# yanjunzan/GMAT

Measured on AMD Instinct MI355X. Metric: SNP-pairs tested/sec (whole node) + GRM GFLOP/s, mouse-sized cohort, higher is better.
Workload: dtype fp6xfp4/fp64

## Files before the change

gmat_amd/_native.py:

```python
import ctypes
import os

import numpy as np

_HERE = os.path.dirname(os.path.abspath(__file__))
LIB_PATH = os.environ.get("GMAT_HIP_LIB", os.path.join(_HERE, "libgmat_hip.so"))

GMAT_AA, GMAT_AD, GMAT_DD = 0, 1, 2
GMAT_GRM_ADD, GMAT_GRM_DOM = 0, 1
GMAT_SCREEN_NONE = -9

_P = ctypes.c_void_p
_I64 = ctypes.c_int64
_D = ctypes.c_double
_INT = ctypes.c_int

_PROTOS = {
    "gmat_last_error": (ctypes.c_char_p, []),
    "gmat_version": (_INT, []),
    "gmat_device_count": (_INT, [_P]),
    "gmat_set_device": (_INT, [_INT]),
    "gmat_device_synchronize": (_INT, []),
    "gmat_empty_cache": (_INT, []),
    "gmat_reml_stats": (_INT, [_P]),
    "gmat_reml_trace": (_INT, [_INT, _P, _P, _P, _P]),
    "gmat_epi_setup_stats": (_INT, [_P, _P]),
    "gmat_geno_create": (_INT, [_P, _P, _I64, _I64, _I64]),
    "gmat_geno_counts": (_INT, [_P, _P, _P, _P]),
    "gmat_geno_destroy": (_INT, [_P]),
    "gmat_grm": (_INT, [_P, _INT, _D, _P, _P]),
    "gmat_grm_stats": (_INT, [_P]),
    "gmat_spd_inverse": (_INT, [_I64, _P, _P, _P]),
    "gmat_reml": (_INT, [_I64, _I64, _I64, _INT, _P, _P, _P, _P, _P, _INT, _D, _D, _P, _P, _P]),
    "gmat_projection": (_INT, [_I64, _I64, _I64, _INT, _P, _P, _P, _P, _P, _P, _P]),
    "gmat_epi_create": (_INT, [_P, _P, _P, _P, _INT]),
    "gmat_epi_create_with": (_INT, [_P, _P, _P, _P, _INT, _P, _I64]),
    "gmat_epi_export": (_INT, [_P, _P, _I64, _P]),
    "gmat_epi_scan": (_INT, [_P, _INT, _P, _I64, _D, _D, _INT, _P]),
    "gmat_epi_hits": (_INT, [_P, _I64, _P, _P, _P, _P, _P, _P]),
    "gmat_epi_pairs": (_INT, [_P, _INT, _P, _I64, _P, _P, _P, _P]),
    "gmat_epi_stats": (_INT, [_P, _P]),
    "gmat_epi_audit": (_INT, [_P, _INT, _P, _I64, _P]),
    "gmat_epi_kernel_stats": (_INT, [_P, _P]),
    "gmat_epi_kernel_stats_ext": (_INT, [_P, _P, _INT, _P]),
    "gmat_epi_info": (_INT, [_P, _P]),
    "gmat_epi_layout": (_INT, [_P, _P]),
    "gmat_epi_destroy": (_INT, [_P]),
    "gmat_eff_scan": (_INT, [_P, _INT, _P, _P, _I64, _P, _P, _P, ctypes.c_char_p, _P]),
    "gmat_eff_stats": (_INT, [_P]),
    "gmat_geno_decode": (_INT, [_P, _P]),
    "gmat_blup": (_INT, [_I64, _I64, _I64, _INT, _P, _P, _P, _P, _P, _P]),
    "gmat_write_grm_text": (_INT, [ctypes.c_char_p, _P, _I64, _INT, ctypes.c_char_p, _INT]),
    "gmat_float_repr": (_INT, [_D, ctypes.c_char_p, _INT]),
    "gmat_append_hit_rows": (_INT, [ctypes.c_char_p, _I64, _P, _P, _INT, _P, _P, _P, _P]),
    "gmat_snp_test": (_INT, [_P, _INT, _P, _P, _P, _P]),
    "gmat_lmm_snp_test": (_INT, [_P, _INT, _P, _P, _I64, _P, _P, _P]),
    "gmat_lmm_epi_rows": (_INT, [_P, _P, _I64, _I64, _P, _P, _P, _P]),
    "gmat_lmm_stats": (_INT, [_P]),
    "gmat_probe_mx_accum":(_INT, [_INT, _P, _P, _P]),
    "gmat_probe_eig_bottom": (_INT, [_I64, _P, _INT, _D, _INT, _P, _P, _P, _P]),
    "gmat_probe_dgemm": (_INT, [_I64, _I64, _I64, _D, _D, _INT, _P, _INT, _INT, _I64, _P, _INT, _INT, _I64, _P, _I64]),
    "gmat_probe_cholesky": (_INT, [_I64, _P, _I64, _INT, _P, _P, _P, _P, _P, _P]),
    "gmat_probe_dot_rows": (_INT, [_I64, _I64, _P, _I64, _P, _I64, _P]),
    "gmat_comm_unique_id": (_INT, [_P]),
    "gmat_comm_init": (_INT, [_P, _INT, _INT, _P]),
    "gmat_comm_destroy": (_INT, [_P]),
    "gmat_comm_allgather": (_INT, [_P, _P, _P, _I64]),
    "gmat_comm_broadcast": (_INT, [_P, _P, _I64, _INT]),
    "gmat_comm_allreduce_f64": (_INT, [_P, _P, _I64, _INT]),
    "gmat_comm_gatherv": (_INT, [_P, _P, _I64, _INT, _P, _P, _I64, _P]),
    "gmat_comm_barrier": (_INT, [_P]),
    "read_plink_bed": (_INT, [ctypes.c_char_p, _I64, _I64, _P]),
    "remma_epiAA_eff_cpu": (_INT, [ctypes.c_char_p, _I64, _I64, _P, _I64, _P, _D, ctypes.c_char_p]),
    "remma_epiAD_eff_cpu": (_INT, [ctypes.c_char_p, _I64, _I64, _P, _I64, _P, _D, ctypes.c_char_p]),
    "remma_epiDD_eff_cpu": (_INT, [ctypes.c_char_p, _I64, _I64, _P, _I64, _P, _D, ctypes.c_char_p]),
# ... 81 lines not shown
```

gmat_amd/csrc/epi.h:

```cpp
#pragma once
#include <algorithm>
#include <chrono>
#include <cmath>
#include <cstring>
#include <numeric>
#include <vector>

#include "dla.h"
#include "geno.h"

namespace gmat {
namespace epi {


typedef int v2i_ __attribute__((ext_vector_type(2)));
typedef int v8i_ __attribute__((ext_vector_type(8)));
typedef float v16f_ __attribute__((ext_vector_type(16)));
typedef float v2f_ __attribute__((ext_vector_type(2)));

constexpr int LK = 64;
constexpr int AP = 80;
constexpr int BJ = 32;
constexpr int ROWS_PER_LAUNCH = 512;
constexpr int LRC_ROWS_PER_LAUNCH = 7168;
// ... 372 lines not shown

constexpr int R8_S = 7, R8_TB = 2048, R8_TILE = R8_S * R8_TB, R8_NC = 32, R8_PP = 128;
constexpr int R8_PP2 = 256;
constexpr int R8_NT = 4;
__host__ __device__ inline int64_t r8_toff(int64_t kb, int64_t NS) {
  const int64_t h = kb >> 1;
  return kb * NS - ((kb & 1) ? h * h : h * (h - 1));
}
__host__ __device__ inline int r8_swz(int r) { return (r & 3) ^ ((r >> 1) & 2); }

inline int seg_max() {
  const char *s = getenv("GMAT_SEG_MAX");
  return s ? std::max(1, std::min(16, atoi(s))) : 8;
}


struct PairArgs {
  const int64_t *ci, *cj;
  int64_t np, n_pad;
  const int8_t *a, *b;
  const _Float16 *Ua, *Ub;
  const double *alpha, *beta;
  const double *qa, *ra, *qb, *rb;
  const double *z, *dg, *py;
  double zz;
  double *side;
  const uint8_t *tiles, *nib_i, *nib_j;
  int64_t tiles_bytes;
  int nK;
  double rho, chi_cut;
  unsigned long long *counter;
  int64_t *oi, *oj;
  double *mpart;
};

__device__ __forceinline__ void pair_test(const PairArgs &x, int64_t p, double M) {
  const double var = M + x.side[p], sw = x.side[4 * x.np + p];
  const double var_lo = var - x.rho * sw - x.side[x.np + p] - 1e-12 * fabs(M);
  const double eff_hi = fabs(x.side[2 * x.np + p]) + x.side[3 * x.np + p];
  if (!(var_lo > 0.0) || eff_hi * eff_hi * (1.0 + 1e-9) >= x.chi_cut * var_lo) {
    const unsigned long long k = atomicAdd(x.counter, 1ULL);
    x.oi[k] = x.ci[p];
    x.oj[k] = x.cj[p];
  }
}

constexpr int PS_PPW = 8;


constexpr int PXR_NK = 16, PXR_NSL = 8;







constexpr int GM = 64, GN = 128, GKK = 64, GPI = 80;





__host__ __device__ inline void fp6_block(const double *v, uint32_t wds[8], double *dq) {
  double mx = 0.0;
  for (int j = 0; j < 32; ++j) mx = fmax(mx, fabs(v[j]));
  int e = -127;
  if (mx > 0.0) {
    e = (int)ceil(log2(mx / 7.5));
    while (ldexp(7.5, e) < mx) ++e;
    while (e > -127 && ldexp(7.5, e - 1) >= mx) --e;
    e = e < -127 ? -127 : e;
  }
  for (int k = 0; k < 8; ++k) wds[k] = 0;
  wds[6] = (uint32_t)(e + 127);
  for (int j = 0; j < 32; ++j) {
    const double y = ldexp(v[j], -e), ay = fabs(y);
    double q;
    uint32_t code;
    if (ay < 2.0) {
// ... 334 lines not shown
                                uint32_t *__restrict__ img);
__global__ void all_pairs_kernel(const int64_t *__restrict__ rows, const int64_t *__restrict__ offs, int64_t m, int tri,
                                 int64_t col_lo, int64_t *__restrict__ pi, int64_t *__restrict__ pj);
__global__ void hit_compact_kernel(int64_t np, const int64_t *__restrict__ pi,
                                                          const int64_t *__restrict__ pj, const double *__restrict__ eff,
                                                          const double *__restrict__ var, const double *__restrict__ chi,
                                                          const double *__restrict__ p, double p_cut,
                                                          unsigned long long *count, int64_t *hi, int64_t *hj,
                                                          double *he, double *hv, double *hc, double *hp);
__global__ void audit_kernel(int64_t n, int64_t n_pad, int R, int ncov, const int8_t *left,
                                                      const int8_t *right, const double *alpha, const double *beta,
                                                      const int64_t *pi, const int64_t *pj, const double *Q,
                                                      const double *U, double pf_mu, double pf_tau, double pf_eps,
                                                      double pf_ku, double lr_lam, double lr_tau, double lr_eps,
                                                      double *out);
__global__ void hit_pack_kernel(int64_t n, const int64_t *ci, const int64_t *cj, const double *eff, const double *var,
                                const double *chi, const double *p, double p_cut, double *out, unsigned long long *count);

constexpr int AUD_T = 256;

enum { KT_PAIR_SIDE = 0, KT_PAIR_MX = 1, KT_REFINE = 2, KT_REFINE_SIDE = 3, KT_N = 4 };
int kt_begin(gmat_epi *e, hipStream_t st, size_t *idx);
int kt_end(gmat_epi *e, hipStream_t st, int kernel, size_t beg, double pairs);
const int8_t *screen_panel(const gmat_epi *e, int which);
const int8_t *screen_sq(const gmat_epi *e, int which);
void kind_codings(int kind, int *lc, int *rc);
int build_coding(gmat_epi *e, int which);
int ensure_rho(gmat_epi *e, int S);
int refine(gmat_epi *e, hipStream_t st, const Coding &L, const Coding &R, const int8_t *lp, const int8_t *rp,
           const int64_t *pi, const int64_t *pj, int64_t np, double *eff, double *var, double *chi, double *p);
bool pair_screen_fits(const gmat_epi *e);
int default_lr_rank(const gmat_epi *e);
int pair_screen(gmat_epi *e, hipStream_t st, const Coding &L, const Coding &R, const int8_t *slp, const int8_t *srp,
                const int64_t *pi, const int64_t *pj, int64_t np, double chi_cut, int64_t *n_out, bool reset = true);
int epi_create_impl(gmat_epi **out, gmat_geno *g, const double *pvp, const double *py, int n_slice,
                    const uint8_t *state, int64_t state_bytes, bool allow_seg = true);
constexpr int64_t EXH_ONLY_NPAD = 8192;
int64_t seg_snps(const gmat_geno *g);
int seg_create(gmat_epi **out, gmat_geno *g, const double *pvp, const double *py, int n_slice, const uint8_t *state,
               int64_t state_bytes);
int scan_dispatch(gmat_epi *e, int kind, const int64_t *rows, int64_t n_rows, double p_cut, double chi_cut, int n_slice,
                  int64_t *n_hits);
int seg_scan(gmat_epi *e, int kind, const int64_t *rows, int64_t n_rows, double p_cut, double chi_cut, int n_slice,
             int64_t *n_hits);
int seg_pairs(gmat_epi *e, int kind, const int64_t *pairs, int64_t n_pairs, double *eff, double *var, double *chi,
              double *p);
int seg_audit(gmat_epi *e, int kind, const int64_t *pairs, int64_t n_pairs, double *out5);
const gmat_epi *seg_base(const gmat_epi *e);
int i8gemm_nt(hipStream_t st, int Z, int M, int N, int K, const int8_t *A, int64_t lda, int64_t za, const int8_t *B,
              int64_t ldb, int64_t zb, int *C, int64_t ldc, int64_t zc);


}
}
```

gmat_amd/csrc/epi_plan.hip:

```cpp
#include "epi.h"

namespace gmat {
namespace epi {

const int8_t *screen_panel(const gmat_epi *e, int which) { return e->spanels.as<int8_t>() + which * e->m * e->n_pad; }

int kt_event(gmat_epi *e, hipStream_t st, size_t *idx) {
  if (e->kev_used == e->kev.size()) {
    hipEvent_t ev;
    GMAT_HIP(hipEventCreate(&ev));
    e->kev.push_back(ev);
  }
  *idx = e->kev_used++;
  GMAT_HIP(hipEventRecord(e->kev[*idx], st));
  return GMAT_OK;
}
int kt_begin(gmat_epi *e, hipStream_t st, size_t *idx) { return kt_event(e, st, idx); }
int kt_end(gmat_epi *e, hipStream_t st, int kernel, size_t beg, double pairs) {
  size_t end;
  GMAT_TRY(kt_event(e, st, &end));
  e->kmarks.push_back({kernel, beg, pairs});
  e->kmarks.push_back({-1, end, 0.0});
  return GMAT_OK;
}
// ... 226 lines not shown
    GMAT_TRY(kt_end(e, st, KT_REFINE, kt0, (double)np));
    GMAT_HIP(hipStreamWaitEvent(st, e->r8ev[1], 0));
    hipLaunchKernelGGL(refine8_fin_kernel, dim3((unsigned)cdiv(np, 256)), dim3(256), 0, st, np, e->r8_terms.as<double>(),
                       L.soff.as<double>(), R.soff.as<double>(), L.qa.as<double>(), L.ra.as<double>(),
                       R.qb.as<double>(), R.rb.as<double>(), e->zz, L.mono.as<uint8_t>(), R.mono.as<uint8_t>(), pi, pj,
                       e->r8_varw.as<double>(), nseg, tpart, e->r8_unit, eff, var, chi, p);
    GMAT_HIP(hipGetLastError());
    return GMAT_OK;
  }
  const int64_t tiles = cdiv(np, RP);
  const int nseg = RF_SEG;
  if (nseg > 1 && e->rf_part.bytes < (size_t)2 * nseg * np * sizeof(double)) {
    GMAT_HIP(hipStreamSynchronize(st));
    GMAT_TRY(e->rf_part.alloc((size_t)2 * nseg * np * sizeof(double)));
  }
  double *epart = nseg > 1 ? e->rf_part.as<double>() : nullptr, *vpart = nseg > 1 ? epart + nseg * np : nullptr;
  hipLaunchKernelGGL(refine_kernel, dim3((unsigned)tiles, (unsigned)nseg), dim3(RT), 0, st, e->n_pad, e->Ps.as<double>(),
                     e->py.as<double>(), lp, rp, L.off.as<double>(), R.off.as<double>(), pi, pj, np, eff, var, epart,
                     vpart);
  GMAT_HIP(hipGetLastError());
  if (nseg > 1) {
    hipLaunchKernelGGL(refine_sum_kernel, dim3((unsigned)cdiv(np, 256)), dim3(256), 0, st, np, nseg, epart, vpart, eff,
                       var);
    GMAT_HIP(hipGetLastError());
  }
  hipLaunchKernelGGL(pvalue_kernel, dim3((unsigned)cdiv(np, 256)), dim3(256), 0, st, np, eff, var, chi, p);
  GMAT_HIP(hipGetLastError());
  return GMAT_OK;
}

bool pair_screen_fits(const gmat_epi *e) { return e->nK <= 63; }
int default_lr_rank(const gmat_epi *e) { return pair_screen_fits(e) && !getenv("GMAT_NO_PAIR_SCREEN") ? 128 : 384; }
int pair_screen(gmat_epi *e, hipStream_t st, const Coding &L, const Coding &R, const int8_t *slp, const int8_t *srp,
                const int64_t *pi, const int64_t *pj, int64_t np, double chi_cut, int64_t *n_out, bool reset) {
  if (n_out) *n_out = 0;
  if (np <= 0 && !n_out) return GMAT_OK;
  if (np <= 0 && reset) return GMAT_OK;
  const int nK = e->nK;
  GMAT_CHECK(nK <= 63, GMAT_E_ARG, "pair screen: %d stages (at most 63: pair_mxw_kernel's squares)", nK);
  GMAT_CHECK(L.U16.p && R.U16.p && L.nibI.p && R.nibJ.p && e->mx_tiles.p && e->z.p && e->dg.p && e->py.p && L.qa.p &&
                 R.qb.p && e->cand2_i.p && e->cand2_j.p && e->counter2.p &&
                 e->cand2_i.bytes >= (size_t)np * 8 && L.U16.bytes >= (size_t)e->m * e->n_pad * 2 &&
                 R.U16.bytes >= (size_t)e->m * e->n_pad * 2 && e->mx_tiles.bytes >= (size_t)nK * nK * MX_TILE,
             GMAT_E_ARG, "pair screen: plan buffers missing (U16 %d %d nib %d %d mx %zu z %d cand2 %zu / %lld counter2 %d)",
             L.U16.p != nullptr, R.U16.p != nullptr, L.nibI.p != nullptr, R.nibJ.p != nullptr, e->mx_tiles.bytes,
             e->z.p != nullptr, e->cand2_i.bytes, (long long)np, e->counter2.p != nullptr);
  if (e->ps_side.bytes < (size_t)5 * np * sizeof(double)) {
    GMAT_HIP(hipStreamSynchronize(st));
    GMAT_TRY(e->ps_side.alloc((size_t)5 * std::max<int64_t>(np, e->cand_cap) * sizeof(double)));
  }
  GMAT_TRY(e->pins.count2.reserve(8));
  PairArgs x;
  x.ci = pi;
  x.cj = pj;
  x.np = np;
  x.n_pad = e->n_pad;
  x.a = slp;
  x.b = srp;
  x.Ua = L.U16.as<_Float16>();
  x.Ub = R.U16.as<_Float16>();
  x.alpha = L.soff.as<double>();
  x.beta = R.soff.as<double>();
  x.qa = L.qa.as<double>();
  x.ra = L.ra.as<double>();
  x.qb = R.qb.as<double>();
  x.rb = R.rb.as<double>();
  x.z = e->z.as<double>();
  x.dg = e->dg.as<double>();
  x.py = e->py.as<double>();
  x.zz = e->zz;
  x.side = e->ps_side.as<double>();
  x.tiles = e->mx_tiles.as<uint8_t>();
  x.nib_i = L.nibI.as<uint8_t>();
  x.nib_j = R.nibJ.as<uint8_t>();
  x.tiles_bytes = (int64_t)e->mx_tiles.bytes;
  x.nK = nK;
  x.rho = e->rho_mx;
  x.chi_cut = chi_cut;
  x.counter = e->counter2.as<unsigned long long>();
  x.oi = e->cand2_i.as<int64_t>();
  x.oj = e->cand2_j.as<int64_t>();
  if (reset) GMAT_HIP(hipMemsetAsync(e->counter2.p, 0, 8, st));
  if (np > 0) {
  static bool attr = false;
  if (!attr) {
    GMAT_HIP(hipFuncSetAttribute((const void *)pair_side_kernel, hipFuncAttributeMaxDynamicSharedMemorySize,
                                 160 * 1024 - 256));
    attr = true;
  }
  size_t kt0;
  GMAT_TRY(kt_begin(e, st, &kt0));
  hipLaunchKernelGGL(pair_side_kernel, dim3((unsigned)cdiv(np, 4 * PS_PPW)), dim3(256),
                     (size_t)3 * e->n_pad * sizeof(float), st, x);
  GMAT_HIP(hipGetLastError());
  GMAT_TRY(kt_end(e, st, KT_PAIR_SIDE, kt0, (double)np));
  GMAT_TRY(kt_begin(e, st, &kt0));
  if (nK <= PXR_NK) {
    if (!e->n_cu) {
      int dev = 0, cus = 0;
      GMAT_HIP(hipGetDevice(&dev));
      GMAT_HIP(hipDeviceGetAttribute(&cus, hipDeviceAttributeMultiprocessorCount, dev));
      e->n_cu = std::max(cus, 8);
    }
    const int64_t wgs = cdiv(np, 256);
    const int nseg = (int)std::max<int64_t>(1, std::min<int64_t>(std::min(seg_max(), nK), e->n_cu / wgs));
    if (nseg > 1 && e->ps_mpart.bytes < (size_t)nseg * np * sizeof(double)) {
      GMAT_HIP(hipStreamSynchronize(st));
      GMAT_TRY(e->ps_mpart.alloc((size_t)std::max(8, nseg) * std::max<int64_t>(np, 1 << 16) * sizeof(double)));
    }
    x.mpart = e->ps_mpart.as<double>();
    hipLaunchKernelGGL(pair_mxr_kernel, dim3((unsigned)wgs, (unsigned)nseg), dim3(512), 0, st, x);
    if (nseg > 1) {
      GMAT_HIP(hipGetLastError());
      hipLaunchKernelGGL(pair_test_kernel, dim3((unsigned)cdiv(np, 256)), dim3(256), 0, st, x, nseg);
    }
  } else {
    const int nQ = cdiv(nK, PXR_NK), nseg = nQ * (nQ + 1) / 2;
    if (e->ps_mpart.bytes < (size_t)nseg * np * sizeof(double)) {
      GMAT_HIP(hipStreamSynchronize(st));
      GMAT_TRY(e->ps_mpart.alloc((size_t)std::max(8, nseg) * std::max<int64_t>(np, 1 << 16) * sizeof(double)));
    }
    x.mpart = e->ps_mpart.as<double>();
    hipLaunchKernelGGL(pair_mxw_kernel, dim3((unsigned)cdiv(np, 256), (unsigned)nseg), dim3(512), 0, st, x);
    GMAT_HIP(hipGetLastError());
    hipLaunchKernelGGL(pair_test_kernel, dim3((unsigned)cdiv(np, 256)), dim3(256), 0, st, x, nseg);
  }
  GMAT_HIP(hipGetLastError());
  GMAT_TRY(kt_end(e, st, KT_PAIR_MX, kt0, (double)np));
  }
  if (!n_out) return GMAT_OK;
  GMAT_HIP(hipMemcpyAsync(e->pins.count2.p, e->counter2.p, 8, hipMemcpyDeviceToHost, st));
  GMAT_HIP(hipStreamSynchronize(st));
  *n_out = (int64_t)*e->pins.count2.as<unsigned long long>();
  return GMAT_OK;
}

void kind_codings(int kind, int *lc, int *rc) {
  *lc = (kind == GMAT_DD) ? 1 : 0;
  *rc = (kind == GMAT_AA) ? 0 : 1;
}


struct Eigen {
  int ne = 0, iters = 0;
  std::vector<double> lam, Z;
  DBuf dZ;
};
int eigen_bottom(gmat_epi *e, const double *dP, double trP, int ne, Eigen *eg) {
  const int64_t n = e->n;
  DBuf A;
  DBuf &Z = eg->dZ;
  GMAT_TRY(A.alloc(n * n * sizeof(double)));
  GMAT_TRY(Z.alloc((size_t)n * ne * sizeof(double)));
  hipLaunchKernelGGL(pf_shift_kernel, dim3((unsigned)cdiv(n * n, 256)), dim3(256), 0, 0, n, dP, 0.0, 4.0 * trP / (double)n,
                     A.as<double>());
  GMAT_HIP(hipGetLastError());
  eg->ne = ne;
  eg->lam.resize(ne);
  eg->Z.resize((size_t)n * ne);
  const char *tenv = getenv("GMAT_EIG_TOL");
  std::vector<double> res(ne);
  GMAT_TRY(sym_eig_bottom(n, A.as<double>(), ne, tenv ? atof(tenv) : 3e-4, 16, eg->lam.data(), Z.as<double>(),
                          res.data(), &eg->iters));
// ... 609 lines not shown
  GMAT_CHECK(kind >= 0 && kind <= 2, GMAT_E_ARG, "gmat_epi_audit: bad kind");
  if (n_pairs == 0) return GMAT_OK;
  if (e->seg) return seg_audit(e, kind, pairs, n_pairs, out5);
  int lc, rc;
  kind_codings(kind, &lc, &rc);
  GMAT_TRY(build_coding(e, lc));
  GMAT_TRY(build_coding(e, rc));
  for (int64_t t = 0; t < n_pairs; ++t)
    GMAT_CHECK(pairs[2 * t] >= 0 && pairs[2 * t] < e->m && pairs[2 * t + 1] >= 0 && pairs[2 * t + 1] < e->m,
               GMAT_E_ARG, "pair %lld out of range", (long long)t);
  std::vector<int64_t> hi(n_pairs), hj(n_pairs);
  for (int64_t t = 0; t < n_pairs; ++t) {
    hi[t] = pairs[2 * t];
    hj[t] = pairs[2 * t + 1];
  }
  DBuf di, dj, dout;
  GMAT_TRY(di.alloc(n_pairs * 8));
  GMAT_TRY(dj.alloc(n_pairs * 8));
  GMAT_TRY(dout.alloc(n_pairs * 5 * 8));
  GMAT_HIP(hipMemcpy(di.p, hi.data(), n_pairs * 8, hipMemcpyHostToDevice));
  GMAT_HIP(hipMemcpy(dj.p, hj.data(), n_pairs * 8, hipMemcpyHostToDevice));
  const int R = e->lr_R > 0 && e->lr_Bs.p ? e->lr_R : 0;
  GMAT_CHECK(R <= AUD_T, GMAT_E_ARG, "gmat_epi_audit: rank %d > %d", R, AUD_T);
  hipLaunchKernelGGL(audit_kernel, dim3((unsigned)n_pairs), dim3(AUD_T), 0, e->s, e->n, e->n_pad, R, e->pf_ncov,
                     screen_panel(e, lc), screen_panel(e, rc), e->code[lc].soff.as<double>(),
                     e->code[rc].soff.as<double>(), di.as<int64_t>(), dj.as<int64_t>(), e->lr_Bs.as<double>(),
                     e->pf_U.as<double>(), e->pf_mu, e->pf_tau, e->pf_eps, e->pf_ku, e->lr_lam, e->lr_tau, e->lr_eps,
                     dout.as<double>());
  GMAT_HIP(hipGetLastError());
  GMAT_HIP(hipMemcpyAsync(out5, dout.p, n_pairs * 5 * 8, hipMemcpyDeviceToHost, e->s));
  GMAT_HIP(hipStreamSynchronize(e->s));
  return GMAT_OK;
}
```

gmat_amd/csrc/epi_refine.hip:

```cpp
#include "epi.h"

namespace gmat {
namespace epi {

__global__ __launch_bounds__(RT, 2) void refine_kernel(int64_t n_pad, const double *__restrict__ P,
                                                       const double *__restrict__ py, const int8_t *left,
                                                       const int8_t *right, const double *alpha, const double *beta,
                                                       const int64_t *pi, const int64_t *pj, int64_t np, double *eff,
                                                       double *var, double *eff_part, double *var_part) {
  __shared__ double As[RK][RM + 1];
  __shared__ double Bs[RK][RP + 1];
  __shared__ double red[4][RP];
  const int tid = threadIdx.x, lane = tid & 63, w = tid >> 6, wm = w >> 1, wn = w & 1;
  const int64_t p0 = (int64_t)blockIdx.x * RP;
  const int ar = tid >> 2, ak = (tid & 3) * 8;
  const int gcol = tid & (RP - 1), gk = (tid >> 7) * 8;
  const int64_t gp = p0 + gcol;
  const bool gval = gp < np;
  const int8_t *gl = gval ? left + pi[gp] * n_pad : left;
  const int8_t *gr = gval ? right + pj[gp] * n_pad : right;
  const double gal = gval ? alpha[pi[gp]] : 0.0, gbe = gval ? beta[pj[gp]] : 0.0;
  double vpart[4] = {0, 0, 0, 0};
  double effp = 0.0;
  v2d_ ra[4];
// ... 452 lines not shown
                                                          const double *soff_l, const double *soff_r, const double *qa,
                                                          const double *ra, const double *qb, const double *rb, double zz,
                                                          const uint8_t *mono_l, const uint8_t *mono_r,
                                                          const int64_t *__restrict__ pi, const int64_t *__restrict__ pj,
                                                          const double *varw, int nseg, const double *tpart, double unit,
                                                          double *eff, double *var, double *chi, double *pv) {
  const int64_t p = (int64_t)blockIdx.x * blockDim.x + threadIdx.x;
  if (p >= np) return;
  const int64_t i = pi[p], j = pj[p];
  const double al = soff_l[i], be = soff_r[j], ab = al * be;
  const double s1 = terms[p], s2 = terms[np + p], s3 = terms[2 * np + p], ef = terms[3 * np + p];
  const double t3 = be * be * qa[i], t5 = al * al * qb[j], t7 = ab * ab * zz, t8 = 2.0 * ab * s2, t4 = -2.0 * ab * be * ra[i],
               t6 = -2.0 * ab * al * rb[j];
  double vw;
  if (nseg > 1) {
    double sum = 0.0;
    for (int s = R8_S - 1; s >= 0; --s) {
      double t = 0.0;
      for (int k = 0; k < nseg; ++k) t += tpart[((int64_t)k * R8_S + s) * np + p];
      sum = sum * (1.0 / 128.0) + t;
    }
    vw = unit * sum;
  } else {
    vw = varw[p];
  }
  const double v = (mono_l[i] || mono_r[j]) ? 0.0 : vw + s3 + 2.0 * s1 + t3 + t5 + t7 + t8 + t4 + t6;
  var[p] = v;
  eff[p] = ef;
  const double cc = ef * ef / v;
  chi[p] = cc;
  pv[p] = (cc < 0.0) ? 1.0 : erfc(sqrt(0.5 * cc));
}

__global__ __launch_bounds__(256) void pair_side_kernel(PairArgs x) {
  extern __shared__ __attribute__((aligned(16))) float zdp[];
  const int64_t n_pad = x.n_pad;
  for (int64_t q = threadIdx.x; q < n_pad; q += blockDim.x) {
    zdp[q] = (float)x.z[q];
    zdp[n_pad + q] = (float)x.dg[q];
    zdp[2 * n_pad + q] = (float)x.py[q];
  }
  __syncthreads();
  const int lane = threadIdx.x & 63, wv = threadIdx.x >> 6;
  for (int k = 0; k < PS_PPW; ++k) {
    const int64_t p = ((int64_t)blockIdx.x * 4 + wv) * PS_PPW + k;
    if (p >= x.np) return;
    const int64_t i = x.ci[p], j = x.cj[p];
    const double dal = x.alpha[i], dbe = x.beta[j], dab = dal * dbe;
    const float al = (float)dal, be = (float)dbe, ab = (float)dab;
    const int8_t *pa = x.a + i * n_pad, *pb = x.b + j * n_pad;
    const _Float16 *ua = x.Ua + i * n_pad, *ub = x.Ub + j * n_pad;
    float s1 = 0, s1a = 0, s2 = 0, s2a = 0, s3 = 0, s3a = 0, ef = 0, efa = 0, sw = 0;
    for (int64_t q0 = 8 * lane; q0 < n_pad; q0 += 512) {
      const v2i_ va = *(const v2i_ *)(pa + q0), vb = *(const v2i_ *)(pb + q0);
      const int8_t *ca = (const int8_t *)&va, *cb = (const int8_t *)&vb;
      typedef _Float16 h8_ __attribute__((ext_vector_type(8)));
      const h8_ u8 = *(const h8_ *)(ua + q0), v8 = *(const h8_ *)(ub + q0);
      float uu[8], vv[8];
#pragma unroll
      for (int t = 0; t < 8; ++t) {
        uu[t] = (float)u8[t];
        vv[t] = (float)v8[t];
      }
      float zz8[8], dd8[8], yy8[8];
      {
        const int o1 = (lane & 8) ? 4 : 0, o2 = 4 - o1;
        const bool sw = lane & 8;
        auto rd2 = [&](const float *base, float *dst) __attribute__((always_inline)) {
          const float4 f1 = *(const float4 *)&base[q0 + o1];
          const float4 f2 = *(const float4 *)&base[q0 + o2];
          *(float4 *)&dst[0] = sw ? f2 : f1;
          *(float4 *)&dst[4] = sw ? f1 : f2;
        };
        rd2(zdp, zz8);
        rd2(zdp + n_pad, dd8);
        rd2(zdp + 2 * n_pad, yy8);
      }
#pragma unroll
      for (int h = 0; h < 8; ++h) {
        const float av = (float)ca[h], bv = (float)cb[h], w = av * bv;
        const float z = zz8[h], d = dd8[h], y = yy8[h];
        const float tu = be * uu[h], tv = al * vv[h], tz = ab * z;
        s1 += w * ((tz - tu) - tv);
        s1a += w * ((fabsf(tu) + fabsf(tv)) + fabsf(tz));
        s2 += av * vv[h];
        s2a += av * fabsf(vv[h]);
        s3 += d * (w * w);
        s3a += fabsf(d) * (w * w);
        const float ey = ((av - al) * (bv - be)) * y;
        ef += ey;
        efa += fabsf(ey);
        sw += w * w;
      }
    }
    double r[9] = {s1, s1a, s2, s2a, s3, s3a, ef, efa, sw};
#pragma unroll
    for (int t = 0; t < 9; ++t)
#pragma unroll
      for (int off = 32; off > 0; off >>= 1) r[t] += __shfl_xor(r[t], off);
    if (lane != 0) continue;
    const double t3 = dbe * dbe * x.qa[i], t5 = dal * dal * x.qb[j], t7 = dab * dab * x.zz, t8 = 2.0 * dab * r[2],
                 t4 = -2.0 * dab * dbe * x.ra[i], t6 = -2.0 * dab * dal * x.rb[j];
    x.side[p] = r[4] + 2.0 * r[0] + t3 + t5 + t7 + t8 + t4 + t6;
    const double fsl = 2.0 * (double)(n_pad / 64 + 8) * 0x1p-24;
    const double su = 2.0 * r[1] + 2.0 * fabs(dab) * r[3];
    x.side[x.np + p] = fsl * (su + r[5]) + 0x1p-10 * su + 0x1p-23 * (fabs(dal) + fabs(dbe)) * 4.0 * (double)n_pad +
                       1e-10 * (r[5] + su + fabs(t3) + fabs(t5) + fabs(t7) + fabs(t4) + fabs(t6));
    x.side[2 * x.np + p] = r[6];
    x.side[3 * x.np + p] = (fsl + 1e-10) * r[7];
    x.side[4 * x.np + p] = r[8];
  }
}

__global__ __launch_bounds__(512, 1) void pair_mxr_kernel(PairArgs x) {
  constexpr int NSL = PXR_NSL, LA = PXR_NSL - 2;
  __shared__ __attribute__((aligned(16))) uint8_t sA[NSL][MX_TILE];
  const int tid = threadIdx.x, lane = tid & 63, h = lane >> 5, c = lane & 31;
  const int w = __builtin_amdgcn_readfirstlane(tid >> 6);
  const int nK = x.nK;
  const int nseg = (int)gridDim.y, seg = (int)blockIdx.y, N_all = nK * (nK + 1) / 2;
  auto toff = [&](int kb) __attribute__((always_inline)) { return kb * nK - kb * (kb - 1) / 2; };
  int kb_lo = 0;
  while (kb_lo < nK && toff(kb_lo) * nseg < N_all * seg) ++kb_lo;
  int kb_hi = kb_lo;
  while (kb_hi < nK && toff(kb_hi) * nseg < N_all * (seg + 1)) ++kb_hi;
  const int N = toff(kb_hi) - toff(kb_lo);
  const int64_t p = (int64_t)blockIdx.x * 256 + 32 * w + c;
  const bool valid = p < x.np;
  v4i wf[2 * PXR_NK];
  {
    const uint8_t *ri = x.nib_i + (valid ? x.ci[p] : 0) * nK * NB_REC, *rj = x.nib_j + (valid ? x.cj[p] : 0) * nK * NB_REC;
#pragma unroll
    for (int g = 0; g < 2 * PXR_NK; ++g) {
      v4i v = {0, 0, 0, 0};
      if (valid && g < 2 * nK) {
        const int s = g >> 1, q = 2 * (g & 1) + h;
        const v4i m1 = *(const v4i *)(ri + s * NB_REC + 16 * q), m2 = *(const v4i *)(ri + s * NB_REC + 64 + 16 * q);
        const v4i s1 = *(const v4i *)(rj + s * NB_REC + 16 * q);
        v = (m1 & s1) | (m2 & (s1 << 1));
      }
      wf[g] = v;
    }
  }
// ... 250 lines not shown
```

gmat_amd/remma/_scan.py:

```python
import ctypes
import functools
import os
import logging
import time

import numpy as np
from scipy.stats import chi2

from .. import _native as N
from .. import dist
from ..plink import count_lines
from ..uvlmm.uvlmm_varcom import projection

KINDS = {"AA": N.GMAT_AA, "AD": N.GMAT_AD, "DD": N.GMAT_DD}
SCAN_HEADER = "snp_0 snp_1 eff chi p_val"
PAIR_HEADER = "snp_0 snp_1 eff var chi p"
N_SLICE = 3



@functools.lru_cache(maxsize=64)
def _chi_cut(p_cut):
    return float(chi2.isf(p_cut, 1)) if p_cut < 1 else 0.0

# ... 18 lines not shown
        self._h = h

    def export_state(self):
        need = ctypes.c_int64()
        N.check(self._lib.gmat_epi_export(self._h, None, 0, ctypes.byref(need)), "gmat_epi_export")
        buf = np.zeros(need.value, dtype=np.uint8)
        N.check(self._lib.gmat_epi_export(self._h, N.ptr(buf), buf.size, ctypes.byref(need)), "gmat_epi_export")
        return buf

    def scan(self, kind, rows, p_cut, n_slice=0):
        rows = N.i64(rows)
        n_hits = ctypes.c_int64()
        chi_cut = _chi_cut(float(p_cut))
        N.check(self._lib.gmat_epi_scan(self._h, KINDS[kind], N.ptr(rows), rows.size, float(p_cut), chi_cut,
                                        int(n_slice), ctypes.byref(n_hits)), "gmat_epi_scan")
        k = n_hits.value
        out = [np.zeros(k, np.int64), np.zeros(k, np.int64)] + [np.zeros(k) for _ in range(4)]
        N.check(self._lib.gmat_epi_hits(self._h, k, *[N.ptr(a) for a in out]), "gmat_epi_hits")
        return tuple(out)

    def pairs(self, kind, pairs):
        pairs = N.i64(np.asarray(pairs).reshape(-1, 2))
        k = pairs.shape[0]
        out = [np.zeros(k) for _ in range(4)]
        N.check(self._lib.gmat_epi_pairs(self._h, KINDS[kind], N.ptr(pairs), k, *[N.ptr(a) for a in out]),
                "gmat_epi_pairs")
        return tuple(out)

    def audit(self, kind, pairs):
        pairs = N.i64(np.asarray(pairs).reshape(-1, 2))
        out = np.zeros((pairs.shape[0], 5))
        N.check(self._lib.gmat_epi_audit(self._h, KINDS[kind], N.ptr(pairs), pairs.shape[0], N.ptr(out)),
                "gmat_epi_audit")
        return out

    def stats(self):
        s = np.zeros(10)
        N.check(self._lib.gmat_epi_stats(self._h, N.ptr(s)), "gmat_epi_stats")
        keys = ("pairs", "candidates", "int8_ops", "screen_s", "refine_s", "side_s", "total_s", "launches",
                "n_slice", "bound_coef")
        return dict(zip(keys, s.tolist()))

    def kernel_stats(self):
        s = np.zeros(8)
        N.check(self._lib.gmat_epi_kernel_stats(self._h, N.ptr(s)), "gmat_epi_kernel_stats")
        keys = ("prefilter_s", "prefilter_launches", "prefilter_ops", "screen_s", "screen_launches", "screen_ops",
                "flush_s", "live_pairs")
        return dict(zip(keys, s.tolist()))

    def kernel_stats_ext(self):
        s = np.zeros(12)
        cnt = ctypes.c_int()
        N.check(self._lib.gmat_epi_kernel_stats_ext(self._h, N.ptr(s), s.size, ctypes.byref(cnt)),
                "gmat_epi_kernel_stats_ext")
        out = {}
        for k, name in enumerate(("pair_side", "pair_mx", "refine", "refine_side")):
            out[name] = {"s": float(s[3 * k]), "launches": float(s[3 * k + 1]), "pairs": float(s[3 * k + 2])}
        return out

    def setup_stats(self):
        s = np.zeros(8)
        N.check(self._lib.gmat_epi_setup_stats(self._h, N.ptr(s)), "gmat_epi_setup_stats")
        keys = ("create_s", "prefilter_cert_s", "eigen_s", "lowrank_cert_s", "slices_bounds_s", "coding_s",
                "cholesky_count", "covariate_directions")
        return dict(zip(keys, s.tolist()))

# ... 203 lines not shown
```

include/gmat_hip.h:

```cpp
#ifndef GMAT_HIP_H
#define GMAT_HIP_H

#include <stdint.h>

#ifdef __cplusplus
extern "C" {
#endif

enum {
  GMAT_OK = 0,
  GMAT_E_ARG = -1,
  GMAT_E_HIP = -2,
  GMAT_E_NOMEM = -3,
  GMAT_E_NOTPD = -4,
  GMAT_E_OVERFLOW = -5,
  GMAT_E_STATE = -6
};

enum { GMAT_AA = 0, GMAT_AD = 1, GMAT_DD = 2 };
enum { GMAT_GRM_ADD = 0, GMAT_GRM_DOM = 1 };

const char *gmat_last_error(void);
int gmat_version(void);
int gmat_device_count(int *n);
// ... 10 lines not shown
int gmat_grm(gmat_geno *g, int kind, double small_val, double *kin, double *scale_out);
int gmat_grm_stats(double *out4);

int gmat_spd_inverse(int64_t n, const double *a, double *ainv, double *logdet);

int gmat_reml(int64_t n_rec, int64_t n_fix, int64_t n_id, int n_gmat, const double *y,
              const double *xmat, const int64_t *z_col, const double *const *gmat, const double *init,
              int maxiter, double cc_par, double cc_gra, double *var_out, int *n_iter, double *history);

int gmat_reml_stats(double *out4);

int gmat_reml_trace(int cap, double *grad_norm, double *update_norm, double *em_weight, int *count);

int gmat_projection(int64_t n_rec, int64_t n_fix, int64_t n_id, int n_gmat, const double *y,
                    const double *xmat, const int64_t *z_col, const double *const *gmat,
                    const double *var_com, double *pvp, double *py);

typedef struct gmat_epi gmat_epi;
int gmat_epi_create(gmat_epi **out, gmat_geno *g, const double *pvp, const double *py, int n_slice);
int gmat_epi_export(const gmat_epi *e, uint8_t *buf, int64_t cap, int64_t *needed);
int gmat_epi_create_with(gmat_epi **out, gmat_geno *g, const double *pvp, const double *py, int n_slice,
                         const uint8_t *state, int64_t state_bytes);
#define GMAT_SCREEN_NONE (-9)
int gmat_epi_scan(gmat_epi *e, int kind, const int64_t *rows, int64_t n_rows, double p_cut, double chi_cut,
                  int n_slice, int64_t *n_hits);
int gmat_epi_hits(gmat_epi *e, int64_t cap, int64_t *i, int64_t *j, double *eff, double *var, double *chi,
                  double *p);
int gmat_epi_pairs(gmat_epi *e, int kind, const int64_t *pairs, int64_t n_pairs, double *eff, double *var,
                   double *chi, double *p);
int gmat_epi_stats(const gmat_epi *e, double *out10);
int gmat_epi_kernel_stats(const gmat_epi *e, double *out8);
int gmat_epi_kernel_stats_ext(const gmat_epi *e, double *out, int cap, int *count);
int gmat_epi_audit(gmat_epi *e, int kind, const int64_t *pairs, int64_t n_pairs, double *out5);
int gmat_epi_info(const gmat_epi *e, double *out8);
int gmat_epi_setup_stats(const gmat_epi *e, double *out8);
int gmat_epi_layout(const gmat_epi *e, int64_t *out4);
int gmat_epi_destroy(gmat_epi *e);

int gmat_blup(int64_t n_rec, int64_t n_fix, int64_t n_id, int n_gmat, const double *y, const double *xmat,
              const int64_t *z_col, const double *const *gmat, const double *var_com, double *rand_eff);

int gmat_eff_scan(gmat_geno *g, int kind, const double *py, const int64_t *rows, int64_t n_rows,
                  const double *eff_cut, const int64_t *freq_i, const int64_t *freq_j, const char *out_file,
                  int64_t *n_hits);
int gmat_eff_stats(double *out4);
int gmat_write_grm_text(const char *path, const double *mat, int64_t n, int fmt, const char *ids_blob, int n_threads);
int gmat_float_repr(double v, char *out, int cap);
int gmat_append_hit_rows(const char *path, int64_t n, const int64_t *i, const int64_t *j, int nf, const double *f0,
                         const double *f1, const double *f2, const double *f3);

int gmat_snp_test(gmat_geno *g, int kind, const double *pvp, const double *py, double *xpy, double *xpx);
int gmat_lmm_snp_test(gmat_geno *g, int mode, const double *p, const double *py, int64_t chunk, double *eff,
                      double *var, double *chi);
int gmat_lmm_epi_rows(gmat_epi *e, const int64_t *rows, int64_t n_rows, int64_t block, double *eff, double *var,
                      double *chi, double *p);
int gmat_lmm_stats(double *out8);

int gmat_geno_decode(const gmat_geno *g, double *marker_mat);

typedef struct gmat_comm gmat_comm;
int gmat_comm_unique_id(uint8_t *out128);
int gmat_comm_init(gmat_comm **out, int nranks, int rank, const uint8_t *id128);
int gmat_comm_destroy(gmat_comm *c);
int gmat_comm_allgather(gmat_comm *c, const void *send, void *recv, int64_t bytes);
int gmat_comm_broadcast(gmat_comm *c, void *buf, int64_t bytes, int root);
int gmat_comm_allreduce_f64(gmat_comm *c, double *v, int64_t count, int op);
// ... 20 lines not shown
```

Baseline: 83.30 billion.

## Group pair-screen side sums by shared row SNP and pack FP32 math

Rewrites pair_side_kernel so each wave processes up to two consecutive candidate pairs that share the same row SNP i together, loading the row's genotype and U vectors once for both pairs. The inner loop uses packed two-wide float FMAs, prefetches the next chunk (software pipelining), and replaces the shuffle-xor reductions with DPP/permlane wave sums. The algebra of the side terms is reorganized (s1 split into separate accumulators and combined in double afterwards), which changes rounding and bound formulas slightly. It also adds a pair-audit entry point and a GMAT_DEBUG run-statistics print, both off the default path.

New measurement: 85.31 billion, median of 6. 1.02x the previous value.

```diff
diff --git a/gmat_amd/_native.py b/gmat_amd/_native.py
--- a/gmat_amd/_native.py
+++ b/gmat_amd/_native.py
@@ -41,6 +41,7 @@
     "gmat_epi_pairs": (_INT, [_P, _INT, _P, _I64, _P, _P, _P, _P]),
     "gmat_epi_stats": (_INT, [_P, _P]),
     "gmat_epi_audit": (_INT, [_P, _INT, _P, _I64, _P]),
+    "gmat_epi_pair_audit": (_INT, [_P, _INT, _P, _I64, _P]),
     "gmat_epi_kernel_stats": (_INT, [_P, _P]),
     "gmat_epi_kernel_stats_ext": (_INT, [_P, _P, _INT, _P]),
     "gmat_epi_info": (_INT, [_P, _P]),
diff --git a/gmat_amd/csrc/epi.h b/gmat_amd/csrc/epi.h
--- a/gmat_amd/csrc/epi.h
+++ b/gmat_amd/csrc/epi.h
@@ -428,12 +428,18 @@
   unsigned long long *counter;
   int64_t *oi, *oj;
   double *mpart;
+  double *audit;
 };
 
 __device__ __forceinline__ void pair_test(const PairArgs &x, int64_t p, double M) {
   const double var = M + x.side[p], sw = x.side[4 * x.np + p];
   const double var_lo = var - x.rho * sw - x.side[x.np + p] - 1e-12 * fabs(M);
   const double eff_hi = fabs(x.side[2 * x.np + p]) + x.side[3 * x.np + p];
+  if (x.audit) {
+    x.audit[p] = var_lo;
+    x.audit[x.np + p] = eff_hi;
+    return;
+  }
   if (!(var_lo > 0.0) || eff_hi * eff_hi * (1.0 + 1e-9) >= x.chi_cut * var_lo) {
     const unsigned long long k = atomicAdd(x.counter, 1ULL);
     x.oi[k] = x.ci[p];
@@ -442,6 +448,7 @@
 }
 
 constexpr int PS_PPW = 8;
+constexpr int PS_G = 2;
 
 
 constexpr int PXR_NK = 16, PXR_NSL = 8;
@@ -842,7 +849,8 @@
 bool pair_screen_fits(const gmat_epi *e);
 int default_lr_rank(const gmat_epi *e);
 int pair_screen(gmat_epi *e, hipStream_t st, const Coding &L, const Coding &R, const int8_t *slp, const int8_t *srp,
-                const int64_t *pi, const int64_t *pj, int64_t np, double chi_cut, int64_t *n_out, bool reset = true);
+                const int64_t *pi, const int64_t *pj, int64_t np, double chi_cut, int64_t *n_out, bool reset = true,
+                double *audit = nullptr);
 int epi_create_impl(gmat_epi **out, gmat_geno *g, const double *pvp, const double *py, int n_slice,
                     const uint8_t *state, int64_t state_bytes, bool allow_seg = true);
 constexpr int64_t EXH_ONLY_NPAD = 8192;
diff --git a/gmat_amd/csrc/epi_plan.hip b/gmat_amd/csrc/epi_plan.hip
--- a/gmat_amd/csrc/epi_plan.hip
+++ b/gmat_amd/csrc/epi_plan.hip
@@ -282,15 +282,16 @@
 bool pair_screen_fits(const gmat_epi *e) { return e->nK <= 63; }
 int default_lr_rank(const gmat_epi *e) { return pair_screen_fits(e) && !getenv("GMAT_NO_PAIR_SCREEN") ? 128 : 384; }
 int pair_screen(gmat_epi *e, hipStream_t st, const Coding &L, const Coding &R, const int8_t *slp, const int8_t *srp,
-                const int64_t *pi, const int64_t *pj, int64_t np, double chi_cut, int64_t *n_out, bool reset) {
+                const int64_t *pi, const int64_t *pj, int64_t np, double chi_cut, int64_t *n_out, bool reset,
+                double *audit) {
   if (n_out) *n_out = 0;
   if (np <= 0 && !n_out) return GMAT_OK;
   if (np <= 0 && reset) return GMAT_OK;
   const int nK = e->nK;
   GMAT_CHECK(nK <= 63, GMAT_E_ARG, "pair screen: %d stages (at most 63: pair_mxw_kernel's squares)", nK);
   GMAT_CHECK(L.U16.p && R.U16.p && L.nibI.p && R.nibJ.p && e->mx_tiles.p && e->z.p && e->dg.p && e->py.p && L.qa.p &&
-                 R.qb.p && e->cand2_i.p && e->cand2_j.p && e->counter2.p &&
-                 e->cand2_i.bytes >= (size_t)np * 8 && L.U16.bytes >= (size_t)e->m * e->n_pad * 2 &&
+                 R.qb.p && (audit || (e->cand2_i.p && e->cand2_j.p && e->counter2.p &&
+                 e->cand2_i.bytes >= (size_t)np * 8)) && L.U16.bytes >= (size_t)e->m * e->n_pad * 2 &&
                  R.U16.bytes >= (size_t)e->m * e->n_pad * 2 && e->mx_tiles.bytes >= (size_t)nK * nK * MX_TILE,
              GMAT_E_ARG, "pair screen: plan buffers missing (U16 %d %d nib %d %d mx %zu z %d cand2 %zu / %lld counter2 %d)",
              L.U16.p != nullptr, R.U16.p != nullptr, L.nibI.p != nullptr, R.nibJ.p != nullptr, e->mx_tiles.bytes,
@@ -330,7 +331,22 @@
   x.counter = e->counter2.as<unsigned long long>();
   x.oi = e->cand2_i.as<int64_t>();
   x.oj = e->cand2_j.as<int64_t>();
-  if (reset) GMAT_HIP(hipMemsetAsync(e->counter2.p, 0, 8, st));
+  x.audit = audit;
+  if (reset && !audit) GMAT_HIP(hipMemsetAsync(e->counter2.p, 0, 8, st));
+  if (np > 0 && !audit && getenv("GMAT_DEBUG")) {
+    std::vector<int64_t> hc(np);
+    GMAT_HIP(hipStreamSynchronize(st));
+    GMAT_HIP(hipMemcpy(hc.data(), pi, np * 8, hipMemcpyDeviceToHost));
+    int64_t runs = 0, groups = 0;
+    for (int64_t t = 0, g = 0; t < np; ++t) {
+      const bool same = t > 0 && hc[t] == hc[t - 1];
+      if (!same || t % 32 == 0) ++runs;
+      g = (same && t % PS_PPW != 0 && g < PS_G) ? g + 1 : 1;
+      if (g == 1) ++groups;
+    }
+    fprintf(stderr, "pair screen: %lld candidates, %lld runs in blocks of 32 (mean %.2f), %lld groups (mean %.2f)\n",
+            (long long)np, (long long)runs, (double)np / runs, (long long)groups, (double)np / groups);
+  }
   if (np > 0) {
   static bool attr = false;
   if (!attr) {
@@ -378,7 +394,7 @@
   GMAT_HIP(hipGetLastError());
   GMAT_TRY(kt_end(e, st, KT_PAIR_MX, kt0, (double)np));
   }
-  if (!n_out) return GMAT_OK;
+  if (!n_out || audit) return GMAT_OK;
   GMAT_HIP(hipMemcpyAsync(e->pins.count2.p, e->counter2.p, 8, hipMemcpyDeviceToHost, st));
   GMAT_HIP(hipStreamSynchronize(st));
   *n_out = (int64_t)*e->pins.count2.as<unsigned long long>();
@@ -1054,3 +1070,40 @@
   GMAT_HIP(hipStreamSynchronize(e->s));
   return GMAT_OK;
 }
+
+extern "C" int gmat_epi_pair_audit(gmat_epi *e, int kind, const int64_t *pairs, int64_t n_pairs, double *out7) {
+  GMAT_CHECK(e && (n_pairs == 0 || (pairs && out7)), GMAT_E_ARG, "gmat_epi_pair_audit: bad arguments");
+  GMAT_CHECK(kind >= 0 && kind <= 2, GMAT_E_ARG, "gmat_epi_pair_audit: bad kind");
+  if (n_pairs == 0) return GMAT_OK;
+  GMAT_CHECK(!e->seg, GMAT_E_ARG, "gmat_epi_pair_audit: not available for a plan split into individual segments");
+  GMAT_CHECK(pair_screen_fits(e), GMAT_E_ARG, "gmat_epi_pair_audit: the pair screen does not run at %d stages", e->nK);
+  int lc, rc;
+  kind_codings(kind, &lc, &rc);
+  GMAT_TRY(build_coding(e, lc));
+  GMAT_TRY(build_coding(e, rc));
+  std::vector<int64_t> hi(n_pairs), hj(n_pairs);
+  for (int64_t t = 0; t < n_pairs; ++t) {
+    hi[t] = pairs[2 * t];
+    hj[t] = pairs[2 * t + 1];
+    GMAT_CHECK(hi[t] >= 0 && hi[t] < e->m && hj[t] >= 0 && hj[t] < e->m, GMAT_E_ARG, "pair %lld out of range",
+               (long long)t);
+  }
+  DBuf di, dj, da;
+  GMAT_TRY(di.alloc(n_pairs * 8));
+  GMAT_TRY(dj.alloc(n_pairs * 8));
+  GMAT_TRY(da.alloc(n_pairs * 2 * 8));
+  GMAT_HIP(hipMemcpy(di.p, hi.data(), n_pairs * 8, hipMemcpyHostToDevice));
+  GMAT_HIP(hipMemcpy(dj.p, hj.data(), n_pairs * 8, hipMemcpyHostToDevice));
+  GMAT_TRY(pair_screen(e, e->s, e->code[lc], e->code[rc], screen_panel(e, lc), screen_panel(e, rc), di.as<int64_t>(),
+                       dj.as<int64_t>(), n_pairs, 1.0, nullptr, false, da.as<double>()));
+  std::vector<double> side((size_t)5 * n_pairs), au((size_t)2 * n_pairs);
+  GMAT_HIP(hipMemcpyAsync(side.data(), e->ps_side.p, side.size() * 8, hipMemcpyDeviceToHost, e->s));
+  GMAT_HIP(hipMemcpyAsync(au.data(), da.p, au.size() * 8, hipMemcpyDeviceToHost, e->s));
+  GMAT_HIP(hipStreamSynchronize(e->s));
+  for (int64_t t = 0; t < n_pairs; ++t) {
+    for (int k = 0; k < 5; ++k) out7[7 * t + k] = side[(size_t)k * n_pairs + t];
+    out7[7 * t + 5] = au[t];
+    out7[7 * t + 6] = au[n_pairs + t];
+  }
+  return GMAT_OK;
+}
diff --git a/gmat_amd/csrc/epi_refine.hip b/gmat_amd/csrc/epi_refine.hip
--- a/gmat_amd/csrc/epi_refine.hip
+++ b/gmat_amd/csrc/epi_refine.hip
@@ -508,6 +508,150 @@
   pv[p] = (cc < 0.0) ? 1.0 : erfc(sqrt(0.5 * cc));
 }
 
+template <int CTRL>
+__device__ __forceinline__ float ps_dpp(float v) {
+  return __int_as_float(__builtin_amdgcn_update_dpp(0, __float_as_int(v), CTRL, 0xf, 0xf, true));
+}
+__device__ __forceinline__ float ps_wave_sum(float r) {
+#pragma clang fp contract(off)
+  r = r + ps_dpp<0xB1>(r);
+  r = r + ps_dpp<0x4E>(r);
+  r = r + ps_dpp<0x141>(r);
+  r = r + ps_dpp<0x140>(r);
+  const auto h = __builtin_amdgcn_permlane16_swap(__float_as_uint(r), __float_as_uint(r), false, false);
+  r = __uint_as_float(h[0]) + __uint_as_float(h[1]);
+  const auto w = __builtin_amdgcn_permlane32_swap(__float_as_uint(r), __float_as_uint(r), false, false);
+  return __uint_as_float(w[0]) + __uint_as_float(w[1]);
+}
+
+template <int G>
+__device__ __forceinline__ void pair_side_group(const PairArgs &x, const float *zdp, int lane, int64_t p0, int64_t i,
+                                                int my_j, int k0) {
+#pragma clang fp contract(off)
+  typedef _Float16 h8_ __attribute__((ext_vector_type(8)));
+  const int64_t n_pad = x.n_pad;
+  const double dal = x.alpha[i];
+  const float al = (float)dal, aal = fabsf(al);
+  const int8_t *pa = x.a + i * n_pad;
+  const _Float16 *ua = x.Ua + i * n_pad;
+  int64_t j[G];
+  const int8_t *pb[G];
+  const _Float16 *ub[G];
+#pragma unroll
+  for (int s = 0; s < G; ++s) {
+    j[s] = __builtin_amdgcn_readfirstlane(__shfl(my_j, k0 + s));
+    pb[s] = x.b + j[s] * n_pad;
+    ub[s] = x.Ub + j[s] * n_pad;
+  }
+  const v2f_ z2 = {0.f, 0.f};
+  v2f_ sA[G], sAa[G], sB[G], sBa[G], s2[G], s2a[G], s3[G], s3a[G], sw[G], ef[G], efa[G];
+#pragma unroll
+  for (int s = 0; s < G; ++s) sA[s] = sAa[s] = sB[s] = sBa[s] = s2[s] = s2a[s] = s3[s] = s3a[s] = sw[s] = ef[s] = efa[s] = z2;
+  v2f_ g5s = z2, g5ms = z2;
+  const v2f_ al2 = {al, al}, aal2 = {aal, aal}, tiny2 = {0x1p-23f, 0x1p-23f};
+  struct Gathered {
+    v2i_ va, vb[G];
+    h8_ u8, v8[G];
+  };
+  auto gather = [&](int64_t q) __attribute__((always_inline)) {
+    Gathered d;
+    d.va = *(const v2i_ *)(pa + q);
+    d.u8 = *(const h8_ *)(ua + q);
+#pragma unroll
+    for (int s = 0; s < G; ++s) {
+      d.vb[s] = *(const v2i_ *)(pb[s] + q);
+      d.v8[s] = *(const h8_ *)(ub[s] + q);
+    }
+    return d;
+  };
+  Gathered nxt = gather(8 * lane < n_pad ? 8 * lane : 0);
+  for (int64_t q0 = 8 * lane; q0 < n_pad; q0 += 512) {
+    const Gathered cur = nxt;
+    nxt = gather(q0 + 512 < n_pad ? q0 + 512 : q0);
+    __builtin_amdgcn_sched_barrier(0);
+    const v2i_ va = cur.va;
+    const h8_ u8 = cur.u8;
+    const v2i_ *vb = cur.vb;
+    const h8_ *v8 = cur.v8;
+    const uint8_t *ca = (const uint8_t *)&va;
+    float zz8[8], dd8[8], yy8[8];
+    {
+      const int o1 = (lane & 8) ? 4 : 0, o2 = 4 - o1;
+      const bool swp = lane & 8;
+      auto rd2 = [&](const float *base, float *dst) __attribute__((always_inline)) {
+        const float4 f1 = *(const float4 *)&base[q0 + o1];
+        const float4 f2 = *(const float4 *)&base[q0 + o2];
+        *(float4 *)&dst[0] = swp ? f2 : f1;
+        *(float4 *)&dst[4] = swp ? f1 : f2;
+      };
+      rd2(zdp, zz8);
+      rd2(zdp + n_pad, dd8);
+      rd2(zdp + 2 * n_pad, yy8);
+    }
+#pragma unroll
+    for (int h = 0; h < 8; h += 2) {
+      const v2f_ av = {(float)ca[h], (float)ca[h + 1]}, uu = {(float)u8[h], (float)u8[h + 1]};
+      const v2f_ z = {zz8[h], zz8[h + 1]}, d = {dd8[h], dd8[h + 1]}, y = {yy8[h], yy8[h + 1]};
+      const v2f_ g1 = av * __builtin_elementwise_fma(al2, z, -uu);
+      const v2f_ g6 = av * __builtin_elementwise_fma(aal2, __builtin_elementwise_abs(z), __builtin_elementwise_abs(uu));
+      const v2f_ g3 = d * (av * av), ag3 = __builtin_elementwise_abs(g3);
+      const v2f_ g5 = (av - al2) * y;
+      const v2f_ g5m = __builtin_elementwise_fma(tiny2, __builtin_elementwise_abs(al2 * y), __builtin_elementwise_abs(g5));
+      g5s = g5s + g5;
+      g5ms = g5ms + g5m;
+#pragma unroll
+      for (int s = 0; s < G; ++s) {
+        const uint8_t *cb = (const uint8_t *)&vb[s];
+        const v2f_ bv = {(float)cb[h], (float)cb[h + 1]}, vv = {(float)v8[s][h], (float)v8[s][h + 1]};
+        const v2f_ avv = __builtin_elementwise_abs(vv);
+        const v2f_ ba = bv * av, b2 = bv * bv;
+        sA[s] = __builtin_elementwise_fma(bv, g1, sA[s]);
+        sAa[s] = __builtin_elementwise_fma(bv, g6, sAa[s]);
+        sB[s] = __builtin_elementwise_fma(ba, vv, sB[s]);
+        sBa[s] = __builtin_elementwise_fma(ba, avv, sBa[s]);
+        s2[s] = __builtin_elementwise_fma(av, vv, s2[s]);
+        s2a[s] = __builtin_elementwise_fma(av, avv, s2a[s]);
+        s3[s] = __builtin_elementwise_fma(b2, g3, s3[s]);
+        s3a[s] = __builtin_elementwise_fma(b2, ag3, s3a[s]);
+        sw[s] = __builtin_elementwise_fma(ba, ba, sw[s]);
+        ef[s] = __builtin_elementwise_fma(bv, g5, ef[s]);
+        efa[s] = __builtin_elementwise_fma(bv, g5m, efa[s]);
+      }
+    }
+  }
+  auto wsum = [](v2f_ v) __attribute__((always_inline)) { return ps_wave_sum(v[0] + v[1]); };
+  auto pick = [&](const v2f_(&acc)[G]) __attribute__((always_inline)) {
+    float r = wsum(acc[0]);
+#pragma unroll
+    for (int s = 1; s < G; ++s) {
+      const float v = wsum(acc[s]);
+      r = lane == s ? v : r;
+    }
+    return (double)r;
+  };
+  const double G5 = (double)wsum(g5s), G5m = (double)wsum(g5ms);
+  const double fsl = 2.0 * (double)(n_pad / 64 + 8) * 0x1p-24;
+  const double r[11] = {pick(sA), pick(sAa), pick(sB), pick(sBa), pick(s2), pick(s2a),
+                        pick(s3), pick(s3a), pick(sw), pick(ef), pick(efa)};
+  int64_t jl = j[0];
+#pragma unroll
+  for (int s = 1; s < G; ++s) jl = lane == s ? j[s] : jl;
+  if (lane < G) {
+    const int64_t p = p0 + lane;
+    const double dbe = x.beta[jl], dab = dal * dbe;
+    const double s1 = dbe * r[0] - dal * r[2], s1a = fabs(dbe) * r[1] + fabs(dal) * r[3];
+    const double t3 = dbe * dbe * x.qa[i], t5 = dal * dal * x.qb[jl], t7 = dab * dab * x.zz, t8 = 2.0 * dab * r[4],
+                 t4 = -2.0 * dab * dbe * x.ra[i], t6 = -2.0 * dab * dal * x.rb[jl];
+    x.side[p] = r[6] + 2.0 * s1 + t3 + t5 + t7 + t8 + t4 + t6;
+    const double su = 2.0 * s1a + 2.0 * fabs(dab) * r[5];
+    x.side[x.np + p] = fsl * (su + r[7]) + 0x1p-10 * su + 0x1p-23 * (fabs(dal) + fabs(dbe)) * 4.0 * (double)n_pad +
+                       1e-10 * (r[7] + su + fabs(t3) + fabs(t5) + fabs(t7) + fabs(t4) + fabs(t6));
+    x.side[2 * x.np + p] = r[9] - dbe * G5;
+    x.side[3 * x.np + p] = (fsl + 1e-10) * (r[10] + fabs(dbe) * G5m);
+    x.side[4 * x.np + p] = r[8];
+  }
+}
+
 __global__ __launch_bounds__(256) void pair_side_kernel(PairArgs x) {
   extern __shared__ __attribute__((aligned(16))) float zdp[];
   const int64_t n_pad = x.n_pad;
@@ -518,73 +662,27 @@
   }
   __syncthreads();
   const int lane = threadIdx.x & 63, wv = threadIdx.x >> 6;
-  for (int k = 0; k < PS_PPW; ++k) {
-    const int64_t p = ((int64_t)blockIdx.x * 4 + wv) * PS_PPW + k;
-    if (p >= x.np) return;
-    const int64_t i = x.ci[p], j = x.cj[p];
-    const double dal = x.alpha[i], dbe = x.beta[j], dab = dal * dbe;
-    const float al = (float)dal, be = (float)dbe, ab = (float)dab;
-    const int8_t *pa = x.a + i * n_pad, *pb = x.b + j * n_pad;
-    const _Float16 *ua = x.Ua + i * n_pad, *ub = x.Ub + j * n_pad;
-    float s1 = 0, s1a = 0, s2 = 0, s2a = 0, s3 = 0, s3a = 0, ef = 0, efa = 0, sw = 0;
-    for (int64_t q0 = 8 * lane; q0 < n_pad; q0 += 512) {
-      const v2i_ va = *(const v2i_ *)(pa + q0), vb = *(const v2i_ *)(pb + q0);
-      const int8_t *ca = (const int8_t *)&va, *cb = (const int8_t *)&vb;
-      typedef _Float16 h8_ __attribute__((ext_vector_type(8)));
-      const h8_ u8 = *(const h8_ *)(ua + q0), v8 = *(const h8_ *)(ub + q0);
-      float uu[8], vv[8];
-#pragma unroll
-      for (int t = 0; t < 8; ++t) {
-        uu[t] = (float)u8[t];
-        vv[t] = (float)v8[t];
-      }
-      float zz8[8], dd8[8], yy8[8];
-      {
-        const int o1 = (lane & 8) ? 4 : 0, o2 = 4 - o1;
-        const bool sw = lane & 8;
-        auto rd2 = [&](const float *base, float *dst) __attribute__((always_inline)) {
-          const float4 f1 = *(const float4 *)&base[q0 + o1];
-          const float4 f2 = *(const float4 *)&base[q0 + o2];
-          *(float4 *)&dst[0] = sw ? f2 : f1;
-          *(float4 *)&dst[4] = sw ? f1 : f2;
-        };
-        rd2(zdp, zz8);
-        rd2(zdp + n_pad, dd8);
-        rd2(zdp + 2 * n_pad, yy8);
-      }
-#pragma unroll
-      for (int h = 0; h < 8; ++h) {
-        const float av = (float)ca[h], bv = (float)cb[h], w = av * bv;
-        const float z = zz8[h], d = dd8[h], y = yy8[h];
-        const float tu = be * uu[h], tv = al * vv[h], tz = ab * z;
-        s1 += w * ((tz - tu) - tv);
-        s1a += w * ((fabsf(tu) + fabsf(tv)) + fabsf(tz));
-        s2 += av * vv[h];
-        s2a += av * fabsf(vv[h]);
-        s3 += d * (w * w);
-        s3a += fabsf(d) * (w * w);
-        const float ey = ((av - al) * (bv - be)) * y;
-        ef += ey;
-        efa += fabsf(ey);
-        sw += w * w;
-      }
-    }
-    double r[9] = {s1, s1a, s2, s2a, s3, s3a, ef, efa, sw};
-#pragma unroll
-    for (int t = 0; t < 9; ++t)
-#pragma unroll
-      for (int off = 32; off > 0; off >>= 1) r[t] += __shfl_xor(r[t], off);
-    if (lane != 0) continue;
-    const double t3 = dbe * dbe * x.qa[i], t5 = dal * dal * x.qb[j], t7 = dab * dab * x.zz, t8 = 2.0 * dab * r[2],
-                 t4 = -2.0 * dab * dbe * x.ra[i], t6 = -2.0 * dab * dal * x.rb[j];
-    x.side[p] = r[4] + 2.0 * r[0] + t3 + t5 + t7 + t8 + t4 + t6;
-    const double fsl = 2.0 * (double)(n_pad / 64 + 8) * 0x1p-24;
-    const double su = 2.0 * r[1] + 2.0 * fabs(dab) * r[3];
-    x.side[x.np + p] = fsl * (su + r[5]) + 0x1p-10 * su + 0x1p-23 * (fabs(dal) + fabs(dbe)) * 4.0 * (double)n_pad +
-                       1e-10 * (r[5] + su + fabs(t3) + fabs(t5) + fabs(t7) + fabs(t4) + fabs(t6));
-    x.side[2 * x.np + p] = r[6];
-    x.side[3 * x.np + p] = (fsl + 1e-10) * r[7];
-    x.side[4 * x.np + p] = r[8];
+  const int64_t pw = ((int64_t)blockIdx.x * 4 + wv) * PS_PPW;
+  if (pw >= x.np) return;
+  const int cnt = (int)min((int64_t)PS_PPW, x.np - pw);
+  int my_i = -1, my_j = 0;
+  if (lane < cnt) {
+    my_i = (int)x.ci[pw + lane];
+    my_j = (int)x.cj[pw + lane];
+  }
+  for (int k = 0; k < cnt;) {
+    const int i = __builtin_amdgcn_readfirstlane(__shfl(my_i, k));
+    int g = 1;
+    while (g < PS_G && k + g < cnt && __builtin_amdgcn_readfirstlane(__shfl(my_i, k + g)) == i) ++g;
+    if (PS_G >= 4 && g == 4)
+      pair_side_group<4>(x, zdp, lane, pw + k, i, my_j, k);
+    else if (PS_G >= 3 && g == 3)
+      pair_side_group<3>(x, zdp, lane, pw + k, i, my_j, k);
+    else if (g == 2)
+      pair_side_group<2>(x, zdp, lane, pw + k, i, my_j, k);
+    else
+      pair_side_group<1>(x, zdp, lane, pw + k, i, my_j, k);
+    k += g;
   }
 }
 
diff --git a/gmat_amd/remma/_scan.py b/gmat_amd/remma/_scan.py
--- a/gmat_amd/remma/_scan.py
+++ b/gmat_amd/remma/_scan.py
@@ -74,6 +74,13 @@
         out = np.zeros((pairs.shape[0], 5))
         N.check(self._lib.gmat_epi_audit(self._h, KINDS[kind], N.ptr(pairs), pairs.shape[0], N.ptr(out)),
                 "gmat_epi_audit")
+        return out
+
+    def pair_audit(self, kind, pairs):
+        pairs = N.i64(np.asarray(pairs).reshape(-1, 2))
+        out = np.zeros((pairs.shape[0], 7))
+        N.check(self._lib.gmat_epi_pair_audit(self._h, KINDS[kind], N.ptr(pairs), pairs.shape[0], N.ptr(out)),
+                "gmat_epi_pair_audit")
         return out
 
     def stats(self):
diff --git a/include/gmat_hip.h b/include/gmat_hip.h
--- a/include/gmat_hip.h
+++ b/include/gmat_hip.h
@@ -66,6 +66,7 @@
 int gmat_epi_kernel_stats(const gmat_epi *e, double *out8);
 int gmat_epi_kernel_stats_ext(const gmat_epi *e, double *out, int cap, int *count);
 int gmat_epi_audit(gmat_epi *e, int kind, const int64_t *pairs, int64_t n_pairs, double *out5);
+int gmat_epi_pair_audit(gmat_epi *e, int kind, const int64_t *pairs, int64_t n_pairs, double *out7);
 int gmat_epi_info(const gmat_epi *e, double *out8);
 int gmat_epi_setup_stats(const gmat_epi *e, double *out8);
 int gmat_epi_layout(const gmat_epi *e, int64_t *out4);
```
